# nihalsid/single-view-3d-reconstruction

Hardware: AMD Instinct MI355X
Metric: query-points/sec fwd+bwd (128^3 grid, 50k pts) (higher is better)
Workload: dtype f32

## Files before the change

### single-view-3d-reconstruction_amd/csrc/gather.hip

```cpp
#include "common.h"
#include "gather_common.h"
#include "reduce.h"

namespace {

struct LevelArgs {
  const float *vol;
  float *gvol;
  int C, D, H, W, col;
  const int32_t *order;
  const int32_t *items;
};

struct FusedArgs {
  LevelArgs L[SVR_MAX_LEVELS];
  unsigned block_start[SVR_MAX_LEVELS + 1];
  int n;
  int pad_start;
  int shared;
  int xcd;
};

template <int C, bool JMAJOR = false>
__device__ __forceinline__ void gather_fwd_body(const LevelArgs L, const float *__restrict__ points,
// ... 495 lines not shown
          fy[s] = c.iy - c.y0f;
          fz[s] = c.iz - c.z0f;
        }
      }
    }
    constexpr int NB = 2 * CW / UNR;
    auto issue = [&](float (&gq)[UNR * CPL], int blk) {
#pragma unroll
      for (int u = 0; u < UNR; ++u) {
        const int t = blk * UNR + u, s = t >= CW ? 1 : 0;
        const int go = bcast(s ? goff[1] : goff[0], grp * CW + t - s * CW);
#pragma unroll
        for (int p = 0; p < CPL; ++p) gq[u * CPL + p] = gfeat[(t < cnt ? go : 0) + cg * CW * CPL + ch + p * CW];
      }
    };
    auto process = [&](const float (&gq)[UNR * CPL], int blk) {
#pragma unroll
      for (int u = 0; u < UNR; ++u) {
        const int t = blk * UNR + u, s = t >= CW ? 1 : 0, src = grp * CW + t - s * CW;
        const int kraw = bcast(s ? key[1] : key[0], src);
        const int bqu = bcast(s ? bb[1] : bb[0], src);
        const float xq = bcastf(s ? fx[1] : fx[0], src), yq = bcastf(s ? fy[1] : fy[0], src),
                    zq = bcastf(s ? fz[1] : fz[0], src);
        const int kk = t < cnt ? kraw : -1;
        if (kk < 0) continue;
        if constexpr (PROJ) {
          if (kk != cur0 || bqu != b0) {
            const bool hand = !STORE && cur0 >= 0 && bqu == b0 && kk == cur0 + 1;
            flush(cur0, b0, acc0, hand ? 0xAA : 0);
            if (hand) {
#pragma unroll
              for (int k = 0; k < 8; k += 2)
#pragma unroll
                for (int p = 0; p < CPL; ++p) { acc0[k * CPL + p] = acc0[(k + 1) * CPL + p]; acc0[(k + 1) * CPL + p] = 0.f; }
            } else {
#pragma unroll
              for (int k = 0; k < 8 * CPL; ++k) acc0[k] = 0.f;
            }
            cur0 = kk;
            b0 = bqu;
            if constexpr (STORE) slot0 = bcast(s ? sid[1] : sid[0], src);
          }
        } else if (kk != cur0 || bqu != b0) {
          if (kk == cur1 && bqu == b1) {
#pragma unroll
            for (int k = 0; k < 8 * CPL; ++k) { const float tt = acc0[k]; acc0[k] = acc1[k]; acc1[k] = tt; }
            cur1 = cur0;
            b1 = b0;
          } else {
            retire();
#pragma unroll
            for (int k = 0; k < 8 * CPL; ++k) { acc1[k] = acc0[k]; acc0[k] = 0.f; }
            cur1 = cur0;
            b1 = b0;
          }
          cur0 = kk;
          b0 = bqu;
        }
        const float wx1 = xq, wx0 = 1.f - wx1, wy1 = yq, wy0 = 1.f - wy1, wz1 = zq, wz0 = 1.f - wz1;
        const float w00 = wy0 * wz0, w10 = wy1 * wz0, w01 = wy0 * wz1, w11 = wy1 * wz1;
        if constexpr (CPL % 2 == 0) {
          typedef float f2 __attribute__((ext_vector_type(2)));
#pragma unroll
          for (int p = 0; p < CPL; p += 2) {
            const f2 g = {gq[u * CPL + p], gq[u * CPL + p + 1]};
            const f2 a00 = g * w00, a10 = g * w10, a01 = g * w01, a11 = g * w11;
#define SVR_ACC2(K, WX, A)                                                                     \
  {                                                                                            \
    const f2 r = __builtin_elementwise_fma(f2{WX, WX}, A, f2{acc0[K * CPL + p], acc0[K * CPL + p + 1]}); \
    acc0[K * CPL + p] = r.x;                                                                   \
    acc0[K * CPL + p + 1] = r.y;                                                               \
  }
            SVR_ACC2(0, wx0, a00) SVR_ACC2(1, wx1, a00) SVR_ACC2(2, wx0, a10) SVR_ACC2(3, wx1, a10)
            SVR_ACC2(4, wx0, a01) SVR_ACC2(5, wx1, a01) SVR_ACC2(6, wx0, a11) SVR_ACC2(7, wx1, a11)
#undef SVR_ACC2
          }
        } else {
#pragma unroll
          for (int p = 0; p < CPL; ++p) {
            const float g = gq[u * CPL + p];
            const float a00 = w00 * g, a10 = w10 * g, a01 = w01 * g, a11 = w11 * g;
            acc0[0 * CPL + p] = __builtin_fmaf(wx0, a00, acc0[0 * CPL + p]); acc0[1 * CPL + p] = __builtin_fmaf(wx1, a00, acc0[1 * CPL + p]);
            acc0[2 * CPL + p] = __builtin_fmaf(wx0, a10, acc0[2 * CPL + p]); acc0[3 * CPL + p] = __builtin_fmaf(wx1, a10, acc0[3 * CPL + p]);
            acc0[4 * CPL + p] = __builtin_fmaf(wx0, a01, acc0[4 * CPL + p]); acc0[5 * CPL + p] = __builtin_fmaf(wx1, a01, acc0[5 * CPL + p]);
            acc0[6 * CPL + p] = __builtin_fmaf(wx0, a11, acc0[6 * CPL + p]); acc0[7 * CPL + p] = __builtin_fmaf(wx1, a11, acc0[7 * CPL + p]);
          }
        }
      }
    };
    float gA[UNR * CPL], gB[UNR * CPL];
    issue(gA, 0);
    for (int blk = 0; blk < NB; blk += 2) {
      if ((blk + 1) * UNR < cnt) issue(gB, blk + 1);
      process(gA, blk);
      if ((blk + 1) * UNR >= cnt) break;
      if ((blk + 2) * UNR < cnt) issue(gA, blk + 2);
      process(gB, blk + 1);
      if ((blk + 2) * UNR >= cnt) break;
    }
  }
  retire();
  flush(cur0, b0, acc0, 0);
}

__host__ __device__ inline int items_cpl(int C) { return C >= 32 ? 2 : 1; }

__global__ __launch_bounds__(256) void gather_bwd_proj_kernel(LevelArgs L, const float *__restrict__ points,
                                                              const float *__restrict__ dh, int64_t T, int N, int lddh,
                                                              float disp, int ac, int64_t waves) {
  const int64_t witem = ((int64_t)blockIdx.x * 256 + threadIdx.x) >> 6;
  gather_bwd_items_body<256, 4, true, kProjReps>(L, points, dh, T, N, lddh, disp, ac, witem, waves);
}

__global__ __launch_bounds__(256) void gather_bwd_proj_store_kernel(LevelArgs L, const float *__restrict__ points,
                                                                    const float *__restrict__ dh, int64_t T, int N, int lddh,
                                                                    float disp, int ac, int64_t waves) {
  const int64_t witem = ((int64_t)blockIdx.x * 256 + threadIdx.x) >> 6;
  gather_bwd_items_body<256, 4, true, kProjReps, true>(L, points, dh, T, N, lddh, disp, ac, witem, waves);
}

__global__ __launch_bounds__(256) void proj_flag_kernel(const uint32_t *__restrict__ keys, int32_t *__restrict__ flags, int64_t T,
                                                        int chunk, uint32_t sentinel) {
  const int64_t i = (int64_t)blockIdx.x * 256 + threadIdx.x;
  if (i > T) return;
  flags[i] = (i < T && keys[i] != sentinel && (i % chunk == 0 || keys[i] != keys[i - 1])) ? 1 : 0;
}

__global__ __launch_bounds__(256) void proj_table_kernel(const uint32_t *__restrict__ keys, const int32_t *__restrict__ sidx,
                                                         int32_t *__restrict__ first_slot, int64_t nkeys, int64_t T) {
  const int64_t q = (int64_t)blockIdx.x * 256 + threadIdx.x;
  if (q > nkeys) return;
  int64_t lo = 0, hi = T;
  while (lo < hi) {
    const int64_t mid = (lo + hi) >> 1;
    if (keys[mid] < (uint32_t)q) lo = mid + 1; else hi = mid;
  }
  first_slot[q] = sidx[lo];
}

__global__ __launch_bounds__(256) void proj_combine_kernel(const float *__restrict__ partials, const int32_t *__restrict__ first_slot,
                                                           float *__restrict__ dP, int B, int D, int H, int W) {
  const int64_t row = (int64_t)blockIdx.x * 4 + (threadIdx.x >> 6);
  const int64_t rows = (int64_t)B * D * H * W * 7;
  if (row >= rows) return;
  const int lane = threadIdx.x & 63;
  const int j = (int)(row % 7);
  int64_t v = row / 7;
  const int x = (int)(v % W);
  v /= W;
  const int y = (int)(v % H);
  v /= H;
  const int z = (int)(v % D);
  const int b = (int)(v / D);
  float4 acc = make_float4(0.f, 0.f, 0.f, 0.f);
#pragma unroll
  for (int k = 0; k < 8; ++k) {
    const int cz = z - (k >> 2) + 1, cy = y - ((k >> 1) & 1) + 1, cx = x - (k & 1) + 1;
    const int64_t q = ((((int64_t)b * (D + 1) + cz) * (H + 1) + cy) * (W + 1) + cx) * 8 + j;
    const int s0 = first_slot[q], s1 = first_slot[q + 1];
    for (int sl = s0; sl < s1; ++sl) {
      const float4 p = *reinterpret_cast<const float4 *>(partials + ((size_t)sl * 8 + k) * 256 + lane * 4);
      acc.x += p.x; acc.y += p.y; acc.z += p.z; acc.w += p.w;
    }
  }
  *reinterpret_cast<float4 *>(dP + row * 256 + lane * 4) = acc;
}

__host__ __device__ inline int64_t bwd_items_waves_cpl(int C, int cpl, int64_t T, int reps = kItemReps) {
  const int cw = (C / cpl) < 64 ? (C / cpl) : 64;
  const int64_t per = (int64_t)(64 / cw) * 2 * cw * reps;
  return svr::cdiv(T, per) * (C / (cw * cpl));
}
__host__ __device__ inline int64_t bwd_items_waves(int C, int64_t T) { return bwd_items_waves_cpl(C, items_cpl(C), T); }

__host__ __device__ inline int64_t bwd_runs_waves(int C, int B, int N) {
  int cw = C < 64 ? C : 64;
  int64_t per = (int64_t)(64 / cw) * 2 * cw;
  int64_t cps = (N + per - 1) / per;
  return cps * B * 7 * (C / cw);
}

__global__ __launch_bounds__(256) void gather_bwd_fused_kernel(FusedArgs A, const float *__restrict__ points,
                                                               const float *__restrict__ gfeat,
                                                               const int32_t *__restrict__ default_order, int B, int N,
                                                               int row_stride, float disp, int ac) {
  int l = 0;
  while (l + 1 < A.n && blockIdx.x >= A.block_start[l + 1]) ++l;
  const LevelArgs L = A.L[l];
  const int64_t item = ((int64_t)(blockIdx.x - A.block_start[l]) * 256 + threadIdx.x) >> 6;
  if (L.items) {
    const int64_t T = (int64_t)7 * B * N, iw = bwd_items_waves(L.C, T);
    switch (L.C) {
      case 16: gather_bwd_items_body<16, 1>(L, points, gfeat, T, N, row_stride, disp, ac, item, iw); break;
      case 32: gather_bwd_items_body<32, 2>(L, points, gfeat, T, N, row_stride, disp, ac, item, iw); break;
      case 64: gather_bwd_items_body<64, 2>(L, points, gfeat, T, N, row_stride, disp, ac, item, iw); break;
      case 128: gather_bwd_items_body<128, 2>(L, points, gfeat, T, N, row_stride, disp, ac, item, iw); break;
    }
    return;
  }
  const int64_t waves = bwd_runs_waves(L.C, B, N);
  const int32_t *order = L.order ? L.order : default_order;
  switch (L.C) {
    case 16: gather_bwd_runs_body<16>(L, points, gfeat, order, B, N, row_stride, disp, ac, item, waves); break;
    case 32: gather_bwd_runs_body<32>(L, points, gfeat, order, B, N, row_stride, disp, ac, item, waves); break;
    case 64: gather_bwd_runs_body<64>(L, points, gfeat, order, B, N, row_stride, disp, ac, item, waves); break;
    case 128: gather_bwd_runs_body<128>(L, points, gfeat, order, B, N, row_stride, disp, ac, item, waves); break;
  }
}

__global__ void corner_index_kernel(const float *__restrict__ points, int32_t *__restrict__ out,
                                    int64_t total, int N, int D, int H, int W, float disp, int ac) {
  int64_t gid = (int64_t)blockIdx.x * blockDim.x + threadIdx.x;
  if (gid >= total) return;
  int n = (int)(gid % N);
  int j = (int)((gid / N) % 7);
  int64_t b = gid / ((int64_t)7 * N);
  Corner c = sample_corner(points + (b * N + n) * 3, j, disp, D, H, W, ac);
  out[gid * 3 + 0] = clamp_int(c.z0f);
  out[gid * 3 + 1] = clamp_int(c.y0f);
  out[gid * 3 + 2] = clamp_int(c.x0f);
}

__global__ __launch_bounds__(128) void gather_bwd_serial_kernel(LevelArgs L, const float *__restrict__ points,
                                                                const float *__restrict__ gfeat, int N,
                                                                int row_stride, float disp, int ac) {
  const int b = blockIdx.x, c = threadIdx.x;
  if (c >= L.C) return;
  float *gb = L.gvol + (size_t)b * L.D * L.H * L.W * L.C + c;
  for (int j = 0; j < 7; ++j)
    for (int n = 0; n < N; ++n) {
      const int64_t pn = (int64_t)b * N + n;
      const Corner cr = sample_corner(points + pn * 3, j, disp, L.D, L.H, L.W, ac);
      const Weights w = corner_weights(cr);
      const float g = gfeat[pn * row_stride + L.col + j * L.C + c];
#pragma unroll
      for (int k = 0; k < 8; ++k) {
        const int z = w.z0 + (k >> 2), y = w.y0 + ((k >> 1) & 1), x = w.x0 + (k & 1);
        if (z >= 0 && z < L.D && y >= 0 && y < L.H && x >= 0 && x < L.W) {
          volatile float *q = gb + (((size_t)z * L.H + y) * L.W + x) * L.C;
          *q = *q + corner_w(w, k) * g;
        }
      }
    }
}

struct PullRec {
  float fx, fy, fz;
  int32_t goff;
};

__device__ __forceinline__ bool pull_cell(const float *pt, int j, float disp, int D, int H, int W, int ac, int b,
                                          uint32_t &key, float &fx, float &fy, float &fz) {
  const Corner c = sample_corner(pt, j, disp, D, H, W, ac);
  const int x0 = clamp_int(c.x0f), y0 = clamp_int(c.y0f), z0 = clamp_int(c.z0f);
  fx = c.ix - c.x0f;
  fy = c.iy - c.y0f;
  fz = c.iz - c.z0f;
  if (!(z0 >= -1 && z0 < D && y0 >= -1 && y0 < H && x0 >= -1 && x0 < W)) return false;
  key = (uint32_t)((((int64_t)b * (D + 1) + z0 + 1) * (H + 1) + y0 + 1) * (W + 1) + x0 + 1);
  return true;
}

__global__ __launch_bounds__(256) void pull_key_kernel(const float *__restrict__ points, uint32_t *__restrict__ keys,
                                                       int32_t *__restrict__ vals, int64_t total, int N, int D, int H,
                                                       int W, float disp, int ac, uint32_t sentinel, int kblk) {
  const int64_t i = (int64_t)blockIdx.x * 256 + threadIdx.x;
  if (i >= total) return;
  const int64_t pn = i / 7;
  const int j = (int)(i - pn * 7);
  uint32_t key;
  float fx, fy, fz;
  const float p3[3] = {points[pn * 3], points[pn * 3 + 1], points[pn * 3 + 2]};
  const bool ok = pull_cell(p3, j, disp, D, H, W, ac, (int)(pn / N), key, fx, fy, fz);
  if (ok && kblk > 0) {
    const uint32_t w1 = (uint32_t)W + 1u, K = (uint32_t)kblk, row = key / w1, x = key - row * w1;
    key = ((row * ((w1 + K - 1u) / K) + x / K) * 8u + (uint32_t)j) * K + x % K;
  }
  keys[i] = ok ? key : sentinel;
  vals[i] = (int32_t)i;
}

__global__ __launch_bounds__(256) void pull_record_kernel(const float *__restrict__ points,
                                                          const uint32_t *__restrict__ keys,
                                                          const int32_t *__restrict__ items, PullRec *__restrict__ recs,
                                                          int32_t *__restrict__ ends, int64_t total, int N, int D, int H,
                                                          int W, int C, int col, int row_stride, float disp, int ac,
                                                          uint32_t sentinel) {
  const int64_t idx = (int64_t)blockIdx.x * 256 + threadIdx.x;
  if (idx >= total) return;
  const uint32_t k = keys[idx];
  if (k == sentinel) return;
  const int32_t id = items[idx];
  const int32_t pn = id / 7;
  const int j = id - pn * 7;
  const float p3[3] = {points[(int64_t)pn * 3], points[(int64_t)pn * 3 + 1], points[(int64_t)pn * 3 + 2]};
  uint32_t key;
  PullRec r;
  pull_cell(p3, j, disp, D, H, W, ac, pn / N, key, r.fx, r.fy, r.fz);
  r.goff = pn * row_stride + col + j * C;
  recs[idx] = r;
  if (idx == total - 1 || keys[idx + 1] != k) ends[k + 1] = (int32_t)idx + 1;
}

template <int C, int XS, int BZ, int BY, int BXG>
__global__ __launch_bounds__(256) void gather_bwd_pull_kernel(float *__restrict__ gvol, const uint32_t *__restrict__ keys,
                                                              const PullRec *__restrict__ recs,
                                                              const int32_t *__restrict__ cs,
                                                              const float *__restrict__ gfeat, int n_items, int B, int D,
                                                              int H, int W) {
  constexpr int V = C / 4;
  static_assert(BZ * BY * BXG * V == 256, "brick must fill the workgroup");
  const int t = threadIdx.x;
  const int q4 = (t % V) * 4, si = t / V;
  const int nbx = (W + BXG * XS - 1) / (BXG * XS), nby = (H + BY - 1) / BY, nbz = (D + BZ - 1) / BZ;
  uint32_t bid = blockIdx.x;
  const int bx = bid % nbx; bid /= nbx;
  const int by = bid % nby; bid /= nby;
  const int bz = bid % nbz;
  const int b = bid / nbz;
  const int x0 = (bx * BXG + si % BXG) * XS, y = by * BY + (si / BXG) % BY, z = bz * BZ + si / (BXG * BY);
  if (x0 >= W || y >= H || z >= D) return;
  const int ncell = min(XS, W - x0) + 1;
  uint32_t kbase[4];
  int lo[4], hi[4];
#pragma unroll
  for (int w = 0; w < 4; ++w) {
    const int dz = w >> 1, dy = w & 1;
    kbase[w] = (uint32_t)((((int64_t)b * (D + 1) + z + dz) * (H + 1) + y + dy) * (W + 1) + x0);
    lo[w] = cs[kbase[w]];
    hi[w] = cs[kbase[w] + ncell];
  }
  float4 acc[XS];
#pragma unroll
  for (int i = 0; i < XS; ++i) acc[i] = make_float4(0.f, 0.f, 0.f, 0.f);
  const int last = n_items - 1;
  while (lo[0] < hi[0] || lo[1] < hi[1] || lo[2] < hi[2] || lo[3] < hi[3]) {
    uint32_t k[4];
    PullRec r[4];
#pragma unroll
    for (int w = 0; w < 4; ++w) {
      const int i = min(lo[w], last);
      k[w] = keys[i];
      r[w] = recs[i];
    }
    float4 g[4];
    bool v[4];
#pragma unroll
    for (int w = 0; w < 4; ++w) {
      v[w] = lo[w] < hi[w];
      g[w] = *reinterpret_cast<const float4 *>(gfeat + (v[w] ? r[w].goff : 0) + q4);
    }
#pragma unroll
    for (int w = 0; w < 4; ++w) {
      const int dz = w >> 1, dy = w & 1;
      if (v[w]) {
        const int o = (int)(k[w] - kbase[w]);
        const float wyz = (dy ? 1.f - r[w].fy : r[w].fy) * (dz ? 1.f - r[w].fz : r[w].fz);
        const float wa = r[w].fx * wyz, wb = (1.f - r[w].fx) * wyz;
#pragma unroll
        for (int i = 0; i < XS; ++i) {
          const float wt = (o == i) ? wa : ((o == i + 1) ? wb : 0.f);
          acc[i].x += wt * g[w].x; acc[i].y += wt * g[w].y; acc[i].z += wt * g[w].z; acc[i].w += wt * g[w].w;
        }
        ++lo[w];
      }
    }
  }
  float *out = gvol + ((((int64_t)b * D + z) * H + y) * W + x0) * C + q4;
#pragma unroll
  for (int i = 0; i < XS; ++i)
    if (x0 + i < W) *reinterpret_cast<float4 *>(out + (int64_t)i * C) = acc[i];
}

template <int XS>
__global__ __launch_bounds__(256) void gather_bwd_pull_c1_kernel(float *__restrict__ gvol, const uint32_t *__restrict__ keys,
                                                                 const PullRec *__restrict__ recs,
                                                                 const int32_t *__restrict__ cs,
                                                                 const float *__restrict__ gfeat, int n_items,
                                                                 int64_t strips, int D, int H, int W) {
  const int64_t t = (int64_t)blockIdx.x * 256 + threadIdx.x;
  if (t >= strips) return;
  const int nsx = (W + XS - 1) / XS;
  const int x0 = (int)(t % nsx) * XS;
  int64_t q = t / nsx;
  const int y = (int)(q % H); q /= H;
  const int z = (int)(q % D);
  const int64_t b = q / D;
  const int ncell = min(XS, W - x0) + 1;
  uint32_t kbase[4];
  int lo[4], hi[4];
#pragma unroll
  for (int w = 0; w < 4; ++w) {
    const int dz = w >> 1, dy = w & 1;
    kbase[w] = (uint32_t)(((b * (D + 1) + z + dz) * (H + 1) + y + dy) * (W + 1) + x0);
    lo[w] = cs[kbase[w]];
    hi[w] = cs[kbase[w] + ncell];
  }
  float acc[XS];
#pragma unroll
  for (int i = 0; i < XS; ++i) acc[i] = 0.f;
  const int last = n_items > 0 ? n_items - 1 : 0;
  while (lo[0] < hi[0] || lo[1] < hi[1] || lo[2] < hi[2] || lo[3] < hi[3]) {
    uint32_t k[4];
    PullRec r[4];
#pragma unroll
    for (int w = 0; w < 4; ++w) {
      const int i = min(lo[w], last);
      k[w] = keys[i];
      r[w] = recs[i];
    }
    float g[4];
    bool v[4];
#pragma unroll
    for (int w = 0; w < 4; ++w) {
      v[w] = lo[w] < hi[w];
      g[w] = gfeat[v[w] ? r[w].goff : 0];
    }
#pragma unroll
    for (int w = 0; w < 4; ++w) {
      const int dz = w >> 1, dy = w & 1;
      if (v[w]) {
        const int o = (int)(k[w] - kbase[w]);
        const float wyz = (dy ? 1.f - r[w].fy : r[w].fy) * (dz ? 1.f - r[w].fz : r[w].fz);
        const float wa = r[w].fx * wyz, wb = (1.f - r[w].fx) * wyz;
#pragma unroll
        for (int i = 0; i < XS; ++i) {
          const float wt = (o == i) ? wa : ((o == i + 1) ? wb : 0.f);
          acc[i] += wt * g[w];
        }
        ++lo[w];
      }
    }
  }
  float *out = gvol + ((b * D + z) * H + y) * (int64_t)W + x0;
#pragma unroll
  for (int i = 0; i < XS; ++i)
    if (x0 + i < W) out[i] = acc[i];
}

__host__ __device__ inline int pull_xs(int C) { return C == 16 ? 8 : 4; }

__global__ __launch_bounds__(256) void pull_stats_kernel(const int32_t *__restrict__ cs, int32_t *__restrict__ stats, int B, int D,
                                                         int H, int W, int XS) {
  const int nsx = (W + XS - 1) / XS;
  const int64_t total = (int64_t)B * (D + 1) * (H + 1) * nsx, i = (int64_t)blockIdx.x * 256 + threadIdx.x;
  int len = 0;
  if (i < total) {
    const int sx = (int)(i % nsx);
    const int64_t row = i / nsx;
    const int x0 = sx * XS, ncell = min(XS, W - x0) + 1;
    const int64_t k = row * (W + 1) + x0;
    len = cs[k + ncell] - cs[k];
  }
  __shared__ int red[256];
  block_max(len, red);
  if (threadIdx.x == 0 && red[0] > 0) atomicMax(stats, red[0]);
}

int64_t pull_cells(int B, int D, int H, int W) { return (int64_t)B * (D + 1) * (H + 1) * (W + 1); }
int pull_key_bits(int64_t cells) {
  int nb = 1;
  while ((1LL << nb) <= cells) ++nb;
  return nb;
}

int check_desc(const svr_gather_desc *d, bool bwd) {
  SVR_CHECK(d != nullptr, SVR_E_BADARG, "gather: null descriptor");
  SVR_CHECK(d->n_levels >= 1 && d->n_levels <= SVR_MAX_LEVELS, SVR_E_BADARG, "gather: n_levels=%d", d->n_levels);
  SVR_CHECK(d->B >= 0 && d->N >= 0, SVR_E_BADSHAPE, "gather: B=%d N=%d", d->B, d->N);
  SVR_CHECK(d->row_stride % 4 == 0, SVR_E_ALIGN, "gather: row_stride %d not a multiple of 4", d->row_stride);
  for (int l = 0; l < d->n_levels; ++l) {
    const svr_level &L = d->level[l];
    SVR_CHECK(L.vol != nullptr || (bwd && L.gvol == nullptr), SVR_E_BADARG, "gather: level %d has no volume", l);
    SVR_CHECK(L.C == 1 || L.C == 16 || L.C == 32 || L.C == 64 || L.C == 128, SVR_E_UNSUPPORTED,
              "gather: level %d: C=%d (supported: 1,16,32,64,128)", l, L.C);
    SVR_CHECK(L.D > 0 && L.H > 0 && L.W > 0, SVR_E_BADSHAPE, "gather: level %d: empty volume", l);
    if (bwd && L.gvol == nullptr && L.vol == nullptr) continue;
    SVR_CHECK(L.col >= 0 && L.col + 7 * L.C <= d->row_stride, SVR_E_BADSHAPE,
              "gather: level %d: columns [%d,%d) exceed row stride %d", l, L.col, L.col + 7 * L.C, d->row_stride);
    SVR_CHECK(L.C == 1 || L.col % 4 == 0, SVR_E_ALIGN, "gather: level %d: col %d not 16-byte aligned", l, L.col);
    SVR_CHECK(((uintptr_t)L.vol & 15) == 0 && ((uintptr_t)L.gvol & 15) == 0, SVR_E_ALIGN,
              "gather: level %d: volume pointer not 16-byte aligned", l);
  }
  return SVR_OK;
}

LevelArgs level_args(const svr_level &L) { return LevelArgs{L.vol, L.gvol, L.C, L.D, L.H, L.W, L.col, L.order, L.item_order}; }

}

#define DISPATCH_C(Cval, ...)                         \
  switch (Cval) {                                     \
    case 1: { constexpr int CC = 1; __VA_ARGS__; } break;     \
    case 16: { constexpr int CC = 16; __VA_ARGS__; } break;   \
    case 32: { constexpr int CC = 32; __VA_ARGS__; } break;   \
    case 64: { constexpr int CC = 64; __VA_ARGS__; } break;   \
    case 128: { constexpr int CC = 128; __VA_ARGS__; } break; \
  }

extern "C" int svr_gather_trilinear_fwd(const svr_gather_desc *d, const float *points, float *features,
                                        void *stream) {
  if (int rc = check_desc(d, false)) return rc;
  if ((int64_t)d->B * d->N == 0) return SVR_OK;
  SVR_CHECK(points && features, SVR_E_BADARG, "gather_fwd: null points/features");
  SVR_CHECK(((uintptr_t)features & 15) == 0, SVR_E_ALIGN, "gather_fwd: features not 16-byte aligned");
  hipStream_t s = (hipStream_t)stream;
  int64_t BN = (int64_t)d->B * d->N;
  if (BN == 0) return SVR_OK;
  FusedArgs A;
  A.n = 0;
  unsigned blocks = 0;
  bool shared = BN * (int64_t)d->row_stride < (1LL << 31) && !(d->flags & SVR_GATHER_WIDE_OFFSETS);
  for (int l = 0; l < d->n_levels; ++l)
    if ((int64_t)d->B * d->level[l].D * d->level[l].H * d->level[l].W * d->level[l].C >= (1LL << 31)) shared = false;
  A.shared = shared ? 1 : 0;
  for (int pass = 0; pass < 2; ++pass)
    for (int l = d->n_levels - 1; l >= 0; --l) {
      if ((d->level[l].C >= 4) != (pass == 0)) continue;
      LevelArgs L = level_args(d->level[l]);
      int V = L.C >= 4 ? L.C / 4 : 1;
      A.L[A.n] = L;
      A.block_start[A.n] = blocks;
      blocks += svr::xcd_grid((shared && L.C >= 16) ? svr::cdiv(BN * 7, 256) : svr::cdiv(BN * 7 * V, 256));
      ++A.n;
    }
  A.block_start[A.n] = blocks;
  static const int xcd_order = getenv("SVR_GATHER_XCD") ? 1 : 0;
  A.xcd = xcd_order;
  A.pad_start = 0;
  for (int l = 0; l < d->n_levels; ++l) {
    int end = d->level[l].col + 7 * d->level[l].C;
    if (end > A.pad_start) A.pad_start = end;
  }
  hipLaunchKernelGGL(gather_fwd_fused_kernel, dim3(blocks), dim3(256), 0, s, A, points, features, d->order, BN, d->N,
                     d->row_stride, d->displacement, d->align_corners);
  return svr::launch_status("gather_fwd");
}

extern "C" int svr_gather_trilinear_bwd(const svr_gather_desc *d, const float *points, const float *gfeatures,
                                        float *gpoints, void *stream) {
  if (int rc = check_desc(d, true)) return rc;
  if ((int64_t)d->B * d->N == 0) return SVR_OK;
  SVR_CHECK(points && gfeatures, SVR_E_BADARG, "gather_bwd: null points/gfeatures");
  hipStream_t s = (hipStream_t)stream;
  int64_t BN = (int64_t)d->B * d->N;
  if (BN == 0) return SVR_OK;
  if (gpoints) {
    hipError_t e = hipMemsetAsync(gpoints, 0, (size_t)BN * 3 * sizeof(float), s);
    SVR_CHECK(e == hipSuccess, (int)e, "gather_bwd: memset failed: %s", hipGetErrorString(e));
  }
  FusedArgs FA;
  FA.n = 0;
  unsigned fblocks = 0;
  for (int l = d->n_levels - 1; l >= 0; --l) {
    LevelArgs L = level_args(d->level[l]);
    bool gv = L.gvol != nullptr;
    if (!gv && !gpoints) continue;
    SVR_CHECK(L.vol != nullptr || !gpoints, SVR_E_BADARG, "gather_bwd: level %d needs vol for the point gradient", l);
    if (gpoints) {
      int V = L.C >= 4 ? L.C / 4 : 1;
      int64_t total = BN * 7 * V;
      unsigned grid = (unsigned)svr::cdiv(total, 256);
      DISPATCH_C(L.C, hipLaunchKernelGGL((gather_bwd_kernel<CC, false, true>), dim3(grid), dim3(256), 0, s, L, points,
                                         gfeatures, gpoints, total, d->N, d->row_stride, d->displacement,
                                         d->align_corners));
    }
    if (!gv) continue;
    if (d->level[l].plan && !(d->flags & SVR_GATHER_DETERMINISTIC)) {
      const svr_pull_plan *P = d->level[l].plan;
      SVR_CHECK(L.C == 1 || L.C == 16 || L.C == 32 || L.C == 64, SVR_E_UNSUPPORTED, "gather_bwd: level %d: pull plan with C=%d", l,
                L.C);
      SVR_CHECK(P->keys && P->recs && P->heads && P->n_items == 7 * BN, SVR_E_BADARG, "gather_bwd: level %d: bad pull plan", l);
      SVR_CHECK(P->n_items < (1LL << 31) && BN * (int64_t)d->row_stride < (1LL << 31), SVR_E_UNSUPPORTED,
                "gather_bwd: level %d: pull plan needs 32-bit item / gradient offsets", l);
      const int n = (int)P->n_items;
      const PullRec *recs = (const PullRec *)P->recs;
#define SVR_PULL(CC, XS, BZ, BY, BXG)                                                                                     \
  {                                                                                                                       \
    const int64_t blocks = (int64_t)d->B * svr::cdiv(L.D, BZ) * svr::cdiv(L.H, BY) * svr::cdiv(L.W, BXG * XS);            \
    SVR_CHECK(blocks < (1LL << 31), SVR_E_UNSUPPORTED, "gather_bwd: level %d: %ld pull workgroups", l, (long)blocks);     \
    hipLaunchKernelGGL((gather_bwd_pull_kernel<CC, XS, BZ, BY, BXG>), dim3((unsigned)blocks), dim3(256), 0, s, L.gvol,    \
                       P->keys, recs, P->heads, gfeatures, n, d->B, L.D, L.H, L.W);                                       \
  }
      if (L.C == 1) {
        const int64_t strips = (int64_t)d->B * L.D * L.H * svr::cdiv(L.W, 4);
        SVR_CHECK(strips < (1LL << 31), SVR_E_UNSUPPORTED, "gather_bwd: level %d: %ld pull strips", l, (long)strips);
        hipLaunchKernelGGL((gather_bwd_pull_c1_kernel<4>), dim3((unsigned)svr::cdiv(strips, 256)), dim3(256), 0, s, L.gvol, P->keys,
                           recs, P->heads, gfeatures, n, strips, L.D, L.H, L.W);
      } else if (L.C == 16) SVR_PULL(16, 8, 4, 4, 4)
      else if (L.C == 32) SVR_PULL(32, 4, 2, 4, 4)
      else SVR_PULL(64, 4, 2, 2, 4)
#undef SVR_PULL
      continue;
    }
    if (d->flags & SVR_GATHER_DETERMINISTIC) {
      hipLaunchKernelGGL(gather_bwd_serial_kernel, dim3((unsigned)d->B), dim3(128), 0, s, L, points, gfeatures, d->N,
                         d->row_stride, d->displacement, d->align_corners);
      continue;
    }
    if (L.C == 1) {
      int64_t total = BN * 7;
      hipLaunchKernelGGL((gather_bwd_kernel<1, true, false>), dim3((unsigned)svr::cdiv(total, 256)), dim3(256), 0, s, L,
                         points, gfeatures, gpoints, total, d->N, d->row_stride, d->displacement, d->align_corners);
      continue;
    }
    FA.L[FA.n] = L;
    FA.block_start[FA.n] = fblocks;
    SVR_CHECK(L.D < 1022 && L.H < 1022 && L.W < 1022, SVR_E_UNSUPPORTED, "gather_bwd: level %d: dims above 1021", l);
    if (L.items) {
      SVR_CHECK(7 * BN < (1LL << 31) && BN * (int64_t)d->row_stride < (1LL << 31), SVR_E_UNSUPPORTED,
                "gather_bwd: level %d: item order needs 32-bit item / gradient offsets", l);
      fblocks += (unsigned)svr::cdiv(bwd_items_waves(L.C, 7 * BN) * 64, 256);
    } else {
      fblocks += (unsigned)svr::cdiv(bwd_runs_waves(L.C, d->B, d->N) * 64, 256);
    }
    ++FA.n;
  }
  if (FA.n > 0) {
    FA.block_start[FA.n] = fblocks;
    hipLaunchKernelGGL(gather_bwd_fused_kernel, dim3(fblocks), dim3(256), 0, s, FA, points, gfeatures, d->order, d->B, d->N,
                       d->row_stride, d->displacement, d->align_corners);
  }
  return svr::launch_status("gather_bwd");
}

extern "C" int svr_gather_corner_indices(const svr_gather_desc *d, int32_t level, const float *points,
                                         int32_t *out, void *stream) {
  if (int rc = check_desc(d, false)) return rc;
  SVR_CHECK(level >= 0 && level < d->n_levels, SVR_E_BADARG, "corner_indices: level %d", level);
  SVR_CHECK(points && out, SVR_E_BADARG, "corner_indices: null pointer");
  const svr_level &L = d->level[level];
  int64_t total = (int64_t)d->B * 7 * d->N;
  if (total == 0) return SVR_OK;
  hipLaunchKernelGGL(corner_index_kernel, dim3((unsigned)svr::cdiv(total, 256)), dim3(256), 0, (hipStream_t)stream,
                     points, out, total, d->N, L.D, L.H, L.W, d->displacement, d->align_corners);
  return svr::launch_status("corner_indices");
}

extern "C" int64_t svr_gather_pull_plan_workspace(int32_t B, int32_t N) {
  const int64_t T = (int64_t)7 * B * N;
  if (T <= 0) return 256;
  return 3 * svr::align256(T * 4) + svr::align256((int64_t)svr::sort_pairs_u32_temp_bytes(T, 32)) + 256;
}

extern "C" int64_t svr_gather_pull_plan_workspace_cells(int32_t B, int32_t D, int32_t H, int32_t W) {
  const int64_t cells = pull_cells(B, D, H, W);
  return svr::align256((cells + 1) * 4) + svr::align256((int64_t)svr::scan_max_i32_temp_bytes(cells + 1)) + 256;
}

extern "C" int svr_gather_pull_plan(const float *points, int32_t B, int32_t N, int32_t D, int32_t H, int32_t W, int32_t C,
                                    int32_t col, int32_t row_stride, int32_t align_corners, float displacement,
                                    uint32_t *keys, void *recs, int32_t *heads, int32_t *items_out, int32_t *stats,
                                    void *workspace, void *stream) {
  const int64_t T = (int64_t)7 * B * N;
  SVR_CHECK(B >= 0 && N >= 0 && D > 0 && H > 0 && W > 0, SVR_E_BADSHAPE, "pull_plan: B=%d N=%d dims %dx%dx%d", B, N, D, H, W);
  SVR_CHECK(heads && workspace, SVR_E_BADARG, "pull_plan: null heads / workspace");
  hipStream_t s = (hipStream_t)stream;
  const int64_t cells = pull_cells(B, D, H, W);
  SVR_CHECK(cells < (1LL << 31) - 1 && T < (1LL << 31) && (int64_t)B * N * row_stride < (1LL << 31), SVR_E_UNSUPPORTED,
            "pull_plan: %ld cells / %ld items / %ld gradient floats exceed 32-bit offsets", (long)cells, (long)T,
            (long)((int64_t)B * N * row_stride));
  char *w = svr::align256(workspace);
  int32_t *ends = (int32_t *)w;
  w += svr::align256((cells + 1) * 4);
  void *scan_tmp = (void *)w;
  const size_t scan_bytes = svr::scan_max_i32_temp_bytes(cells + 1);
  w += svr::align256((int64_t)scan_bytes);
  hipError_t e = hipMemsetAsync(ends, 0, (size_t)(cells + 1) * sizeof(int32_t), s);
  SVR_CHECK(e == hipSuccess, (int)e, "pull_plan: memset failed: %s", hipGetErrorString(e));
  if (T > 0) {
    SVR_CHECK(points && keys && recs, SVR_E_BADARG, "pull_plan: null pointer");
    uint32_t *keys_in = (uint32_t *)w;
    w += svr::align256(T * 4);
    int32_t *vals_in = (int32_t *)w;
    w += svr::align256(T * 4);
    int32_t *items = items_out ? items_out : (int32_t *)w;
    w += svr::align256(T * 4);
    const uint32_t sentinel = (uint32_t)cells;
    const int bits = pull_key_bits(cells);
    hipLaunchKernelGGL(pull_key_kernel, dim3((unsigned)svr::cdiv(T, 256)), dim3(256), 0, s, points, keys_in, vals_in, T, N, D,
                       H, W, displacement, align_corners, sentinel, 0);
    e = svr::sort_pairs_u32((void *)w, svr::sort_pairs_u32_temp_bytes(T, bits), keys_in, keys, vals_in, items, T, bits, s);
    SVR_CHECK(e == hipSuccess, (int)e, "pull_plan: radix sort failed: %s", hipGetErrorString(e));
    hipLaunchKernelGGL(pull_record_kernel, dim3((unsigned)svr::cdiv(T, 256)), dim3(256), 0, s, points, keys, items,
                       (PullRec *)recs, ends, T, N, D, H, W, C, col, row_stride, displacement, align_corners, sentinel);
  }
  e = svr::scan_max_i32(scan_tmp, scan_bytes, ends, heads, cells + 1, s);
  SVR_CHECK(e == hipSuccess, (int)e, "pull_plan: scan failed: %s", hipGetErrorString(e));
  if (stats) {
    e = hipMemsetAsync(stats, 0, 2 * sizeof(int32_t), s);
    SVR_CHECK(e == hipSuccess, (int)e, "pull_plan: memset failed: %s", hipGetErrorString(e));
    const int XS = pull_xs(C);
    const int64_t strips = (int64_t)B * (D + 1) * (H + 1) * svr::cdiv(W, XS);
    hipLaunchKernelGGL(pull_stats_kernel, dim3((unsigned)svr::cdiv(strips, 256)), dim3(256), 0, s, (const int32_t *)heads, stats, B,
                       D, H, W, XS);
  }
  return svr::launch_status("pull_plan");
}

namespace {
int item_order_impl(const float *points, int32_t B, int32_t N, int32_t D, int32_t H, int32_t W, int32_t align_corners,
                    float displacement, int32_t kblk, int32_t *items, void *workspace, void *stream) {
  const int64_t T = (int64_t)7 * B * N;
  SVR_CHECK(B >= 0 && N >= 0 && D > 0 && H > 0 && W > 0, SVR_E_BADSHAPE, "item_order: B=%d N=%d dims %dx%dx%d", B, N, D, H, W);
  SVR_CHECK(kblk >= 0 && kblk <= W + 1, SVR_E_BADARG, "item_order: block length %d outside [1, W + 1 = %d]", kblk, W + 1);
  if (T == 0) return SVR_OK;
  SVR_CHECK(points && items && workspace, SVR_E_BADARG, "item_order: null pointer");
  const int64_t cells = pull_cells(B, D, H, W);
  const int64_t nkeys = kblk ? (int64_t)B * (D + 1) * (H + 1) * svr::cdiv((int64_t)W + 1, (int64_t)kblk) * 8 * kblk : cells;
  SVR_CHECK(nkeys < (1LL << 31) - 1 && T < (1LL << 31), SVR_E_UNSUPPORTED, "item_order: %ld keys / %ld items exceed 32 bits",
            (long)nkeys, (long)T);
  hipStream_t s = (hipStream_t)stream;
  char *w = svr::align256(workspace);
  uint32_t *keys_in = (uint32_t *)w;
  w += svr::align256(T * 4);
  int32_t *vals_in = (int32_t *)w;
  w += svr::align256(T * 4);
  uint32_t *keys_out = (uint32_t *)w;
  w += svr::align256(T * 4);
  const int bits = pull_key_bits(nkeys);
  hipLaunchKernelGGL(pull_key_kernel, dim3((unsigned)svr::cdiv(T, 256)), dim3(256), 0, s, points, keys_in, vals_in, T, N, D, H,
                     W, displacement, align_corners, (uint32_t)nkeys, kblk);
  hipError_t e = svr::sort_pairs_u32((void *)w, svr::sort_pairs_u32_temp_bytes(T, bits), keys_in, keys_out, vals_in, items, T,
                                     bits, s);
  SVR_CHECK(e == hipSuccess, (int)e, "item_order: radix sort failed: %s", hipGetErrorString(e));
  return svr::launch_status("item_order");
}
}

extern "C" int svr_gather_item_order(const float *points, int32_t B, int32_t N, int32_t D, int32_t H, int32_t W,
                                     int32_t align_corners, float displacement, int32_t with_j, int32_t *items,
                                     void *workspace, void *stream) {
  return item_order_impl(points, B, N, D, H, W, align_corners, displacement, with_j ? 1 : 0, items, workspace, stream);
}

extern "C" int svr_gather_item_order_xblock(const float *points, int32_t B, int32_t N, int32_t D, int32_t H, int32_t W,
// ... 89 lines not shown
```

Before: 26.42 million.

## Restructure backward pull walk with record prefetch and DPP quad sharing

Factors the per-strip pull loop of the gather backward kernels into a PullWalk helper. It precomputes a fixed trip count, so the while-loop condition over four ranges is gone. For the C-channel kernel it loads the next round's key and record ahead of time, so those loads overlap the current accumulation. When C<=32 it has each lane of a quad load only one wall's record and shares the four records across the quad with DPP moves, which cuts redundant global loads. The cost is more register pressure and a dependence on quad lanes having the expected wall mapping; inline asm barriers pin the load and compute ordering.

```diff
diff --git a/single-view-3d-reconstruction_amd/csrc/gather.hip b/single-view-3d-reconstruction_amd/csrc/gather.hip
--- a/single-view-3d-reconstruction_amd/csrc/gather.hip
+++ b/single-view-3d-reconstruction_amd/csrc/gather.hip
@@ -821,6 +821,112 @@
   if (idx == total - 1 || keys[idx + 1] != k) ends[k + 1] = (int32_t)idx + 1;
 }
 
+typedef int pull_i4 __attribute__((ext_vector_type(4), aligned(4)));
+__device__ __forceinline__ void pull_ldg(float4 &g, const float *p) { g = *reinterpret_cast<const float4 *>(p); }
+__device__ __forceinline__ void pull_ldg(float &g, const float *p) { g = *p; }
+__device__ __forceinline__ void pull_mad(float4 &a, float wt, const float4 &g) {
+  a.x += wt * g.x; a.y += wt * g.y; a.z += wt * g.z; a.w += wt * g.w;
+}
+__device__ __forceinline__ void pull_mad(float &a, float wt, float g) { a += wt * g; }
+
+template <typename G>
+struct PullRound {
+  int o[4];
+  float wa[4], wb[4];
+  G g[4];
+};
+
+struct PullWalk {
+  const uint32_t *keys;
+  const PullRec *recs;
+  const float *gsrc;
+  uint32_t kbase[4], lo[4], last;
+  int cnt[4];
+  uint32_t k[4];
+  pull_i4 rec[4];
+  uint32_t my_lo;
+
+  template <bool SHARED>
+  __device__ __forceinline__ void load_records(int r) {
+    if constexpr (SHARED) {
+      const uint32_t i = min(my_lo + (uint32_t)r, last);
+      k[0] = keys[i];
+      rec[0] = *reinterpret_cast<const pull_i4 *>(recs + i);
+    } else {
+#pragma unroll
+      for (int w = 0; w < 4; ++w) {
+        const uint32_t i = min(lo[w] + (uint32_t)r, last);
+        k[w] = keys[i];
+        rec[w] = *reinterpret_cast<const pull_i4 *>(recs + i);
+      }
+    }
+  }
+  template <int CTRL>
+  __device__ __forceinline__ static int quad(int v) { return __builtin_amdgcn_mov_dpp(v, CTRL, 0xf, 0xf, false); }
+  __device__ __forceinline__ void exchange() {
+    const int kk = (int)k[0];
+    const pull_i4 m = rec[0];
+    k[0] = quad<0x00>(kk); k[1] = quad<0x55>(kk); k[2] = quad<0xAA>(kk); k[3] = quad<0xFF>(kk);
+#pragma unroll
+    for (int c = 0; c < 4; ++c) {
+      rec[0][c] = quad<0x00>(m[c]); rec[1][c] = quad<0x55>(m[c]); rec[2][c] = quad<0xAA>(m[c]); rec[3][c] = quad<0xFF>(m[c]);
+    }
+  }
+  template <bool SHARED, typename G>
+  __device__ __forceinline__ void issue(PullRound<G> &R, int r) {
+    if constexpr (SHARED) exchange();
+#pragma unroll
+    for (int w = 0; w < 4; ++w) pull_ldg(R.g[w], gsrc + (r < cnt[w] ? rec[w].w : 0));
+#pragma unroll
+    for (int w = 0; w < 4; ++w) {
+      const int dz = w >> 1, dy = w & 1;
+      const float fx = __int_as_float(rec[w].x), fy = __int_as_float(rec[w].y), fz = __int_as_float(rec[w].z);
+      const float wyz = (dy ? 1.f - fy : fy) * (dz ? 1.f - fz : fz);
+      R.o[w] = (int)(k[w] - kbase[w]);
+      R.wa[w] = fx * wyz;
+      R.wb[w] = (1.f - fx) * wyz;
+      asm volatile("" : "+v"(R.o[w]), "+v"(R.wa[w]), "+v"(R.wb[w]));
+    }
+  }
+  __device__ __forceinline__ void pin_loads() const { asm volatile("" ::"s"(keys), "s"(recs), "v"(gsrc) : "memory"); }
+  template <int XS, typename G>
+  __device__ __forceinline__ void accumulate(G (&acc)[XS], const PullRound<G> &R, int r) const {
+#pragma unroll
+    for (int w = 0; w < 4; ++w)
+      if (r < cnt[w]) {
+        const int o = R.o[w];
+        const float wa = R.wa[w], wb = R.wb[w];
+#pragma unroll
+        for (int i = 0; i < XS; ++i) {
+          const float wt = (o == i) ? wa : ((o == i + 1) ? wb : 0.f);
+          pull_mad(acc[i], wt, R.g[w]);
+        }
+      }
+  }
+  template <int XS, int AHEAD, bool SHARED, typename G>
+  __device__ __forceinline__ void run(G (&acc)[XS], const int32_t *cs, int ncell, int n_items) {
+#pragma unroll
+    for (int w = 0; w < 4; ++w) {
+      lo[w] = (uint32_t)cs[kbase[w]];
+      cnt[w] = cs[kbase[w] + ncell] - (int)lo[w];
+    }
+    const int n = max(max(cnt[0], cnt[1]), max(cnt[2], cnt[3]));
+    if (n <= 0) return;
+    last = (uint32_t)n_items - 1u;
+    const int q = threadIdx.x & 3;
+    my_lo = q == 0 ? lo[0] : q == 1 ? lo[1] : q == 2 ? lo[2] : lo[3];
+    PullRound<G> R;
+    if (AHEAD) load_records<SHARED>(0);
+    for (int r = 0; r < n; ++r) {
+      if (!AHEAD) load_records<SHARED>(r);
+      issue<SHARED>(R, r);
+      if (AHEAD) load_records<SHARED>(r + 1);
+      pin_loads();
+      accumulate<XS>(acc, R, r);
+    }
+  }
+};
+
 template <int C, int XS, int BZ, int BY, int BXG>
 __global__ __launch_bounds__(256) void gather_bwd_pull_kernel(float *__restrict__ gvol, const uint32_t *__restrict__ keys,
                                                               const PullRec *__restrict__ recs,
@@ -840,51 +946,17 @@
   const int x0 = (bx * BXG + si % BXG) * XS, y = by * BY + (si / BXG) % BY, z = bz * BZ + si / (BXG * BY);
   if (x0 >= W || y >= H || z >= D) return;
   const int ncell = min(XS, W - x0) + 1;
-  uint32_t kbase[4];
-  int lo[4], hi[4];
+  PullWalk wk;
+  wk.keys = keys; wk.recs = recs; wk.gsrc = gfeat + q4;
 #pragma unroll
   for (int w = 0; w < 4; ++w) {
     const int dz = w >> 1, dy = w & 1;
-    kbase[w] = (uint32_t)((((int64_t)b * (D + 1) + z + dz) * (H + 1) + y + dy) * (W + 1) + x0);
-    lo[w] = cs[kbase[w]];
-    hi[w] = cs[kbase[w] + ncell];
+    wk.kbase[w] = (uint32_t)((((int64_t)b * (D + 1) + z + dz) * (H + 1) + y + dy) * (W + 1) + x0);
   }
   float4 acc[XS];
 #pragma unroll
   for (int i = 0; i < XS; ++i) acc[i] = make_float4(0.f, 0.f, 0.f, 0.f);
-  const int last = n_items - 1;
-  while (lo[0] < hi[0] || lo[1] < hi[1] || lo[2] < hi[2] || lo[3] < hi[3]) {
-    uint32_t k[4];
-    PullRec r[4];
-#pragma unroll
-    for (int w = 0; w < 4; ++w) {
-      const int i = min(lo[w], last);
-      k[w] = keys[i];
-      r[w] = recs[i];
-    }
-    float4 g[4];
-    bool v[4];
-#pragma unroll
-    for (int w = 0; w < 4; ++w) {
-      v[w] = lo[w] < hi[w];
-      g[w] = *reinterpret_cast<const float4 *>(gfeat + (v[w] ? r[w].goff : 0) + q4);
-    }
-#pragma unroll
-    for (int w = 0; w < 4; ++w) {
-      const int dz = w >> 1, dy = w & 1;
-      if (v[w]) {
-        const int o = (int)(k[w] - kbase[w]);
-        const float wyz = (dy ? 1.f - r[w].fy : r[w].fy) * (dz ? 1.f - r[w].fz : r[w].fz);
-        const float wa = r[w].fx * wyz, wb = (1.f - r[w].fx) * wyz;
-#pragma unroll
-        for (int i = 0; i < XS; ++i) {
-          const float wt = (o == i) ? wa : ((o == i + 1) ? wb : 0.f);
-          acc[i].x += wt * g[w].x; acc[i].y += wt * g[w].y; acc[i].z += wt * g[w].z; acc[i].w += wt * g[w].w;
-        }
-        ++lo[w];
-      }
-    }
-  }
+  wk.run<XS, 1, (C <= 32)>(acc, cs, ncell, n_items);
   float *out = gvol + ((((int64_t)b * D + z) * H + y) * W + x0) * C + q4;
 #pragma unroll
   for (int i = 0; i < XS; ++i)
@@ -906,51 +978,17 @@
   const int z = (int)(q % D);
   const int64_t b = q / D;
   const int ncell = min(XS, W - x0) + 1;
-  uint32_t kbase[4];
-  int lo[4], hi[4];
+  PullWalk wk;
+  wk.keys = keys; wk.recs = recs; wk.gsrc = gfeat;
 #pragma unroll
   for (int w = 0; w < 4; ++w) {
     const int dz = w >> 1, dy = w & 1;
-    kbase[w] = (uint32_t)(((b * (D + 1) + z + dz) * (H + 1) + y + dy) * (W + 1) + x0);
-    lo[w] = cs[kbase[w]];
-    hi[w] = cs[kbase[w] + ncell];
+    wk.kbase[w] = (uint32_t)(((b * (D + 1) + z + dz) * (H + 1) + y + dy) * (W + 1) + x0);
   }
   float acc[XS];
 #pragma unroll
   for (int i = 0; i < XS; ++i) acc[i] = 0.f;
-  const int last = n_items > 0 ? n_items - 1 : 0;
-  while (lo[0] < hi[0] || lo[1] < hi[1] || lo[2] < hi[2] || lo[3] < hi[3]) {
-    uint32_t k[4];
-    PullRec r[4];
-#pragma unroll
-    for (int w = 0; w < 4; ++w) {
-      const int i = min(lo[w], last);
-      k[w] = keys[i];
-      r[w] = recs[i];
-    }
-    float g[4];
-    bool v[4];
-#pragma unroll
-    for (int w = 0; w < 4; ++w) {
-      v[w] = lo[w] < hi[w];
-      g[w] = gfeat[v[w] ? r[w].goff : 0];
-    }
-#pragma unroll
-    for (int w = 0; w < 4; ++w) {
-      const int dz = w >> 1, dy = w & 1;
-      if (v[w]) {
-        const int o = (int)(k[w] - kbase[w]);
-        const float wyz = (dy ? 1.f - r[w].fy : r[w].fy) * (dz ? 1.f - r[w].fz : r[w].fz);
-        const float wa = r[w].fx * wyz, wb = (1.f - r[w].fx) * wyz;
-#pragma unroll
-        for (int i = 0; i < XS; ++i) {
-          const float wt = (o == i) ? wa : ((o == i + 1) ? wb : 0.f);
-          acc[i] += wt * g[w];
-        }
-        ++lo[w];
-      }
-    }
-  }
+  wk.run<XS, 0, false>(acc, cs, ncell, n_items);
   float *out = gvol + ((b * D + z) * H + y) * (int64_t)W + x0;
 #pragma unroll
   for (int i = 0; i < XS; ++i)
```

After: 26.59 million (median of 6 runs). Within noise of the previous version (+0.6%).
